# djukic14/BlockSparseMatrices.jl

Hardware: AMD Instinct MI355X
Metric: fp64 block-SpMV GB/s (VBCRS mul!, algorithmic bytes / time) (higher is better)
Workload: dtype f64

## Files before the change

blocksparsematrices.jl_amd/csrc/bsm_analysis.cpp:

```cpp
#include "bsm_analysis.h"

#include <algorithm>
#include <cassert>
#include <chrono>
#include <cmath>
#include <cstdio>
#include <cstdlib>
#include <cstring>
#include <numeric>
#include <set>
#include <thread>
#include <tuple>
#include <unordered_map>

namespace bsm {

Tunables Tunables::from_env() {
    Tunables t;
    auto geti = [](const char *name, int64_t dflt) -> int64_t {
        const char *s = std::getenv(name);
        if (!s || !*s) return dflt;
        return std::strtoll(s, nullptr, 10);
    };
    t.split2_bytes = geti("BSM_SPLIT2_BYTES", t.split2_bytes);
// ... 207 lines not shown
struct Item {
    int64_t group;
    int64_t s_begin, s_end;
    int64_t bytes;
    int nw;
    int32_t color;
};

struct C64h {
    float re, im;
};
struct C128h {
    double re, im;
};
template <typename U> inline const U &stored(const U &v) { return v; }
inline float stored(double v) { return (float)v; }
inline C64h stored(const C128h &v) { return C64h{(float)v.re, (float)v.im}; }

template <typename U, typename V = U>
void pack_chunk_perm(const V *src, int64_t ld, int ra, int mc, int64_t n, const int32_t *dstpos, int E,
                     bool trans, U *dst) {
    for (int64_t w = 0; w < n; w++) {
        const int64_t mp = dstpos[w];
        U *d = dst + ((mp / E) * mc) * E + (mp % E);
        if (!trans) {
            const V *col = src + ra + w * ld;
            for (int i = 0; i < mc; i++) d[(int64_t)i * E] = stored(col[i]);
        } else {
            const V *row = src + w + (int64_t)ra * ld;
            for (int i = 0; i < mc; i++) d[(int64_t)i * E] = stored(row[(int64_t)i * ld]);
        }
    }
}

template <typename U, typename V = U>
void pack_chunk(const V *src, int64_t ld, int ra, int mc, int64_t n, int64_t woff, int E, bool trans,
                U *dst) {
    const int64_t s_first = woff / E, s_last = (woff + n - 1) / E;
    for (int64_t s = s_first; s <= s_last; s++) {
        const int64_t w0 = s * E - woff;
        const int e_lo = (int)std::max<int64_t>(0, -w0);
        const int e_hi = (int)std::min<int64_t>(E, n - w0);
        U *d = dst + (s * mc) * E;
        if (!trans) {
            for (int e = e_lo; e < e_hi; e++) {
                const V *col = src + ra + (w0 + e) * ld;
                for (int i = 0; i < mc; i++) d[(int64_t)i * E + e] = stored(col[i]);
            }
        } else {
            for (int i = 0; i < mc; i++) {
                const V *row = src + w0 + (int64_t)(ra + i) * ld;
                for (int e = e_lo; e < e_hi; e++) d[(int64_t)i * E + e] = stored(row[e]);
            }
        }
    }
}

struct U16 {
    uint64_t a, b;
};

uint64_t hash_list(const int64_t *p, int64_t n) {
    uint64_t h = 0xcbf29ce484222325ull ^ (uint64_t)n;
    for (int64_t i = 0; i < n; i++) {
        h ^= (uint64_t)p[i];
        h *= 0x100000001b3ull;
        h ^= h >> 29;
    }
    return h;
}

}

namespace {
int64_t count_scale_waves(const std::vector<uint8_t> &cover, int64_t own_lo, int64_t own_hi);
}

struct Analysis::BuildState {
    bool sym = false;
    bool colored = false;
    int64_t nb = 0;
    int64_t own_lo = 0, own_hi = 0;
    std::vector<Chunk> chunks;
    std::vector<Group> groups;
    std::vector<const int64_t *> glist;
    std::vector<int32_t> colpos;
    std::vector<uint8_t> ckind;
    std::vector<uint8_t> group_perm;
    std::vector<int64_t> layout;
    uint64_t val_units = 0;
    std::vector<uint8_t> cover;
    std::vector<int32_t> group_color;
    int32_t ncolors_fused = 1;
    std::vector<Item> items;
    bool use_window = false;
    std::unordered_map<uint64_t, int32_t> cuts;
    std::vector<int64_t> item_wg;
    int64_t nwg_items = 0;
    std::vector<int64_t> wg_perm;
};

std::string Analysis::build(int mtype_, int dtype_, int64_t nrows_, int64_t ncols_,
                            const std::vector<BlockIn> &blocks, const AnalysisOptions &opt_) {
    mtype = mtype_;
    dtype = dtype_;
    nrows = nrows_;
    ncols = ncols_;
    opt = opt_;
    tun = Tunables::from_env();
    const bool timing = std::getenv("BSM_TIMING") != nullptr;
    auto t_last = std::chrono::steady_clock::now();
    auto lap = [&](const char *what) {
        if (!timing) return;
        auto now = std::chrono::steady_clock::now();
        std::fprintf(stderr, "[bsm analysis] %-28s %8.1f ms\n", what,
                     std::chrono::duration<double, std::milli>(now - t_last).count());
        t_last = now;
    };
    BuildState st;
    std::string err = stage_validate(blocks, st);
    if (!err.empty()) return err;
    lap("validate");
    bool colour_oom = false;
    if (opt.meta_only) {
        reference_colourings(blocks, colour_oom);
        return colour_oom ? "out of host memory (colouring)" : "";
    }
    if (!(err = stage_row_groups(blocks, st)).empty()) return err;
    if (!(err = stage_merge_columns(blocks, st)).empty()) return err;
    lap("groups + column lists");
    if (!(err = stage_accumulation(blocks, st)).empty()) return err;
    lap("exclusivity / fused colours");
    std::thread colour_thread([&] { reference_colourings(blocks, colour_oom); });
    struct Joiner {
        std::thread &t;
        ~Joiner() {
            if (t.joinable()) t.join();
        }
    } colour_join{colour_thread};
    stage_work_items(st);
    if (plan_cuts(st)) {
        if (!(err = stage_row_groups(blocks, st)).empty()) return err;
        if (!(err = stage_merge_columns(blocks, st)).empty()) return err;
        if (!(err = stage_accumulation(blocks, st)).empty()) return err;
        stage_work_items(st);
        assert(st.nwg_items + (count_scale_waves(st.cover, st.own_lo, st.own_hi) + kWavesPerWg - 1) / kWavesPerWg <= resident_capacity());
        lap("row cuts: groups again");
    }
    stage_dispatch_order(st);
    stage_place_values(st);
    lap("work items + value placement");
    if (!(err = stage_pack_values(blocks, st)).empty()) return err;
    lap("pack values");
    stage_waves(st);
    stage_windows(st);
    if (!(err = stage_gather_index(st)).empty()) return err;
    lap("schedule");
    colour_thread.join();
    lap("reference colourings (tail not hidden by packing)");
    if (colour_oom) return "out of host memory (colouring)";
    return "";
}

std::string Analysis::stage_validate(const std::vector<BlockIn> &blocks, BuildState &st) {
    static const int kEs[6] = {4, 8, 8, 16, 4, 8};
    static const int kVs[6] = {4, 8, 8, 16, 8, 16};
    if (dtype < 0 || dtype > 5) return "unknown dtype";
    es = kEs[dtype];
    vs = kVs[dtype];
    E = 16 / es;
    if (nrows < 0 || ncols < 0) return "negative matrix size";
    if (nrows > INT32_MAX - 64 || ncols > INT32_MAX - 64) return "matrix dimension exceeds int32 range";
    const int64_t nb = st.nb = (int64_t)blocks.size();
    bool sym = (mtype == MT_SYMMETRIC);
    for (const BlockIn &B : blocks) sym |= (B.kind != KIND_PLAIN);
    st.sym = sym;
    st.own_lo = (opt.own_lo > 0) ? opt.own_lo - 1 : 0;
    st.own_hi = (opt.own_hi > 0) ? std::min(opt.own_hi, nrows) : nrows;
    const int64_t rlim = sym ? std::min(nrows, ncols) : nrows;
    const int64_t clim = sym ? std::min(nrows, ncols) : ncols;

    nnz = 0;
    stored_entries = 0;
    int64_t idx_meta = 0;
    for (int64_t b = 0; b < nb; b++) {
        const BlockIn &B = blocks[b];
        if (B.m < 0 || B.n < 0) return "block " + std::to_string(b + 1) + ": negative size";
        if (B.m > 0 && B.n > 0 && !B.data) return "block " + std::to_string(b + 1) + ": null data";
        if (B.ld < std::max<int64_t>(B.trans ? B.n : B.m, 1))
            return "block " + std::to_string(b + 1) + ": ld < m";
        if (B.m > 0 && !B.ridx && (B.r0 < 1 || B.r0 + B.m - 1 > rlim))
            return "block " + std::to_string(b + 1) + ": row range outside matrix";
        if (B.n > 0 && !B.cidx && (B.c0 < 1 || B.c0 + B.n - 1 > clim))
            return "block " + std::to_string(b + 1) + ": column range outside matrix";
        if (opt.validate) {
            if (B.ridx)
                for (int64_t i = 0; i < B.m; i++)
                    if (B.ridx[i] < 1 || B.ridx[i] > rlim)
                        return "block " + std::to_string(b + 1) + ": row index out of range";
            if (B.cidx)
                for (int64_t i = 0; i < B.n; i++)
                    if (B.cidx[i] < 1 || B.cidx[i] > clim)
                        return "block " + std::to_string(b + 1) + ": column index out of range";
        }
        stored_entries += B.m * B.n;
        nnz += (B.kind == KIND_OFF ? 2 : 1) * B.m * B.n;
        idx_meta += (B.kind == KIND_DIAG) ? B.m : (B.m + B.n);
    }
    {
        int64_t meta;
        if (mtype == MT_VBCRS)
            meta = 8 * ((int64_t)rowptr.size() + (int64_t)rowindices.size() + 4 * nb);
        else
            meta = 8 * idx_meta;
        alg_bytes = stored_entries * es + meta + ncols * vs + nrows * vs;
    }

    return "";
}

void Analysis::reference_colourings(const std::vector<BlockIn> &blocks, bool &colour_oom) {
    const int64_t nb = (int64_t)blocks.size();
    {
        try {
            for (auto &c : colors) c.clear();
            if (opt.skip_colors) return;
            auto refcolor = [&](const std::vector<const int64_t *> &l, const std::vector<int64_t> &n) {
                return opt.coloring == 1 ? color_dsatur(l, n) : color_workstream_dsatur(l, n);
            };
            auto single = [](int64_t n) {
                std::vector<std::vector<int64_t>> out(1);
                out[0].resize(n);
                std::iota(out[0].begin(), out[0].end(), (int64_t)1);
                return out;
            };
            if (mtype == MT_BLOCKSPARSE) {
                if (opt.scheduler == 0) {
                    colors[0] = single(nb);
                    colors[1] = single(nb);
                } else {
                    std::vector<const int64_t *> rl(nb), cl(nb);
                    std::vector<int64_t> rn(nb), cn(nb);
                    for (int64_t b = 0; b < nb; b++) {
                        rl[b] = blocks[b].ridx;
                        rn[b] = blocks[b].ridx ? blocks[b].m : 0;
                        cl[b] = blocks[b].cidx;
                        cn[b] = blocks[b].cidx ? blocks[b].n : 0;
                    }
                    colors[0] = refcolor(rl, rn);
                    colors[1] = refcolor(cl, cn);
                }
            } else if (mtype == MT_SYMMETRIC) {
                std::vector<const int64_t *> dl, rl, cl;
                std::vector<int64_t> dn, rn, cn;
                for (const BlockIn &B : blocks) {
                    if (B.kind == KIND_DIAG) {
                        dl.push_back(B.ridx);
                        dn.push_back(B.ridx ? B.m : 0);
                    } else {
                        rl.push_back(B.ridx);
                        rn.push_back(B.ridx ? B.m : 0);
                        cl.push_back(B.cidx);
                        cn.push_back(B.cidx ? B.n : 0);
                    }
                }
                colors[0] = refcolor(rl, rn);
                colors[1] = refcolor(cl, cn);
                colors[2] = refcolor(dl, dn);
            }
        } catch (const std::bad_alloc &) {
            colour_oom = true;
        }
    }
}

std::string Analysis::stage_row_groups(const std::vector<BlockIn> &blocks, BuildState &st) {
    const int64_t nb = st.nb;
    auto &chunks = st.chunks;
    auto &groups = st.groups;
    auto &glist = st.glist;
    const int chunk_rows = tun.chunk_rows;
    std::unordered_map<uint64_t, std::vector<int64_t>> gmap;

    chunks.clear();
    groups.clear();
    glist.clear();
    rows.clear();
    cols.clear();
    for (int64_t b = 0; b < nb; b++) {
        const BlockIn &B = blocks[b];
        if (B.m == 0 || B.n == 0) continue;
        for (int64_t ra0 = 0; ra0 < B.m; ra0 += chunk_rows) {
            const int mc0 = (int)std::min<int64_t>(chunk_rows, B.m - ra0);
            int cut_h = mc0;
            if (!st.cuts.empty() && B.kind == KIND_PLAIN) {
                bool contig = true;
                if (B.ridx)
                    for (int i = 1; i < mc0 && contig; i++) contig = B.ridx[ra0 + i] == B.ridx[ra0] + i;
                if (contig) {
                    const int64_t rb = (B.ridx ? B.ridx[ra0] : B.r0 + ra0) - 1;
                    auto it = st.cuts.find(((uint64_t)rb << 8) | (uint64_t)mc0);
                    if (it != st.cuts.end()) cut_h = it->second;
                }
            }
            for (int64_t ra = ra0; ra < ra0 + mc0; ra += cut_h) {
                const int mc = (int)std::min<int64_t>(cut_h, ra0 + mc0 - ra);
                bool rcontig = true;
// ... 385 lines not shown
        }
        if (best == load[a]) break;
        const int64_t d = cost[mine[a][bi]] - cost[mine[bc][bj]];
        std::swap(mine[a][bi], mine[bc][bj]);
        load[a] -= d;
        load[bc] += d;
    }
    st.wg_perm.assign((size_t)nwg, -1);
    for (size_t c = 0; c < (size_t)ncus; c++) {
        std::stable_sort(mine[c].begin(), mine[c].end(), [&](int64_t a, int64_t b) { return cost[a] > cost[b]; });
        for (size_t i = 0; i < mine[c].size(); i++) st.wg_perm[(size_t)slots[c][i]] = mine[c][i];
    }
}

void Analysis::stage_place_values(BuildState &st) {
    auto &groups = st.groups;
    std::vector<uint8_t> placed(groups.size(), 0);
    st.layout.clear();
    st.layout.reserve(groups.size());
    std::vector<const Item *> order;
    order.reserve(st.items.size());
    if (st.wg_perm.empty()) {
        for (const Item &it : st.items) order.push_back(&it);
    } else {
        std::vector<std::vector<const Item *>> of_wg(st.wg_perm.size());
        for (size_t i = 0; i < st.items.size(); i++) of_wg[(size_t)st.item_wg[i]].push_back(&st.items[i]);
        for (int64_t w : st.wg_perm) order.insert(order.end(), of_wg[(size_t)w].begin(), of_wg[(size_t)w].end());
    }
    for (const Item *it : order)
        if (!placed[it->group]) {
            placed[it->group] = 1;
            st.layout.push_back(it->group);
        }
    for (size_t g = 0; g < groups.size(); g++)
        if (!placed[g]) st.layout.push_back((int64_t)g);
    uint64_t off = 0;
    for (int64_t g : st.layout) {
        groups[g].val_off = off;
        off += (uint64_t)groups[g].mc * (uint64_t)groups[g].strips;
    }
}

std::string Analysis::stage_pack_values(const std::vector<BlockIn> &blocks, BuildState &st) {
    auto &chunks = st.chunks;
    auto &groups = st.groups;
    auto &colpos = st.colpos;
    auto &group_perm = st.group_perm;
    const uint64_t val_units = st.val_units;

    auto pack_one = [&](const Chunk &c, char *dst) {
        const BlockIn &B = blocks[c.blk];
        if (group_perm[c.group]) {
            const int32_t *dp = colpos.data() + groups[c.group].col_off + c.woff;
            if (dtype == 4)
                pack_chunk_perm<float, double>((const double *)B.data, B.ld, c.ra, c.mc, B.n, dp, E, B.trans, (float *)dst);
            else if (dtype == 5)
                pack_chunk_perm<C64h, C128h>((const C128h *)B.data, B.ld, c.ra, c.mc, B.n, dp, E, B.trans, (C64h *)dst);
            else if (es == 4)
                pack_chunk_perm<uint32_t>((const uint32_t *)B.data, B.ld, c.ra, c.mc, B.n, dp, E, B.trans, (uint32_t *)dst);
            else if (es == 8)
                pack_chunk_perm<uint64_t>((const uint64_t *)B.data, B.ld, c.ra, c.mc, B.n, dp, E, B.trans, (uint64_t *)dst);
            else
                pack_chunk_perm<U16>((const U16 *)B.data, B.ld, c.ra, c.mc, B.n, dp, E, B.trans, (U16 *)dst);
            return;
        }
        if (dtype == 4)
            pack_chunk<float, double>((const double *)B.data, B.ld, c.ra, c.mc, B.n, c.woff, E, B.trans, (float *)dst);
        else if (dtype == 5)
            pack_chunk<C64h, C128h>((const C128h *)B.data, B.ld, c.ra, c.mc, B.n, c.woff, E, B.trans, (C64h *)dst);
        else if (es == 4)
            pack_chunk<uint32_t>((const uint32_t *)B.data, B.ld, c.ra, c.mc, B.n, c.woff, E, B.trans, (uint32_t *)dst);
        else if (es == 8)
            pack_chunk<uint64_t>((const uint64_t *)B.data, B.ld, c.ra, c.mc, B.n, c.woff, E, B.trans, (uint64_t *)dst);
        else
            pack_chunk<U16>((const U16 *)B.data, B.ld, c.ra, c.mc, B.n, c.woff, E, B.trans, (U16 *)dst);
    };
    auto pack_many = [&](const std::vector<int32_t> *ids, size_t nchunks, char *base, size_t wbase) {
        const int nt = (int)std::max<int64_t>(1, std::min<int64_t>(tun.pack_threads, (int64_t)nchunks / 64 + 1));
        auto worker = [&](int t) {
            for (size_t k = t; k < nchunks; k += nt) {
                const Chunk &c = chunks[ids ? (size_t)(*ids)[k] : k];
                pack_one(c, base + ((size_t)groups[c.group].val_off * 16 - wbase));
            }
        };
        std::vector<std::thread> th;
        for (int t = 1; t < nt; t++) th.emplace_back(worker, t);
        worker(0);
        for (auto &x : th) x.join();
    };
    auto zero_tail = [&](const Group &G, char *base, size_t wbase) {
        if (G.strips * E - G.width > 0)
            std::memset(base + (((size_t)G.val_off + (size_t)(G.strips - 1) * G.mc) * 16 - wbase), 0, (size_t)G.mc * 16);
    };
    bool streamed = false;
    pack_plan.clear();
    pack_colpos.clear();
    if (opt.blocks_on_device) {
        pack_plan.reserve(chunks.size());
        bool any_perm = false;
        for (const Chunk &c : chunks) {
            const BlockIn &B = blocks[c.blk];
            PackChunk pc;
            pc.src = (uint64_t)(uintptr_t)B.data;
            pc.dst_unit = groups[c.group].val_off;
            pc.ld = B.ld;
            pc.ra = c.ra;
            pc.mc = c.mc;
            pc.n = (int32_t)B.n;
            pc.woff = (int32_t)c.woff;
            pc.perm_off = group_perm[c.group] ? (int32_t)(groups[c.group].col_off + c.woff) : -1;
            pc.trans = B.trans ? 1 : 0;
            any_perm |= pc.perm_off >= 0;
            pack_plan.push_back(pc);
        }
        if (any_perm) pack_colpos = colpos;
    } else if (opt.sink) {
        std::string err = opt.sink->begin((size_t)value_bytes, &streamed);
        if (!err.empty()) return err;
    }
    if (opt.blocks_on_device) {
    } else if (streamed) {
        const std::vector<int64_t> &lay = st.layout;
        std::vector<int32_t> ids;
        size_t g0 = 0;
        while (g0 < lay.size()) {
            const size_t wbase = (size_t)groups[lay[g0]].val_off * 16;
            size_t g1 = g0, wbytes = 0;
            while (g1 < lay.size() && (g1 == g0 || wbytes + (size_t)groups[lay[g1]].mc * groups[lay[g1]].strips * 16 <= tun.window_bytes)) {
                wbytes += (size_t)groups[lay[g1]].mc * (size_t)groups[lay[g1]].strips * 16;
                g1++;
            }
            char *buf = opt.sink->window(wbytes);
            if (!buf) return "value sink: no staging buffer";
            ids.clear();
            for (size_t g = g0; g < g1; g++) {
                zero_tail(groups[lay[g]], buf, wbase);
                ids.insert(ids.end(), groups[lay[g]].chunks.begin(), groups[lay[g]].chunks.end());
            }
            pack_many(&ids, ids.size(), buf, wbase);
            std::string err = opt.sink->commit(wbase, wbytes);
            if (!err.empty()) return err;
            g0 = g1;
        }
        std::string err = opt.sink->end();
        if (!err.empty()) return err;
    } else {
        values.allocate((size_t)val_units * 16);
        for (const Group &G : groups) zero_tail(G, values.data(), 0);
        pack_many(nullptr, chunks.size(), values.data(), 0);
    }
    return "";
}

void Analysis::stage_waves(BuildState &st) {
    auto &groups = st.groups;
    auto &ckind = st.ckind;
    auto &cover = st.cover;
    auto &items = st.items;
    const bool colored = st.colored;
    const int32_t ncolors_fused = st.ncolors_fused;
    const int64_t own_lo = st.own_lo, own_hi = st.own_hi;

    waves.clear();
    std::vector<WaveWork> *nop_out = &waves;
    auto emit_nop = [&]() {
        WaveWork w;
        std::memset(&w, 0, sizeof w);
        w.work = WORK_NOP;
        w.grp = 1;
        w.rbase = -1;
        nop_out->push_back(w);
    };
    color_wg_ptr.clear();
    int32_t cur_color = -1;
    std::vector<WaveWork> *out = &waves;
    auto item_waves = [&](const Item &it) {
        std::vector<WaveWork> &waves = *out;
        while ((int)(waves.size() % kWavesPerWg) % it.nw != 0) emit_nop();
        const Group &G = groups[it.group];
        const int64_t total = it.s_end - it.s_begin;
        const int64_t per_wave = (total + it.nw - 1) / it.nw;
        for (int w = 0; w < it.nw; w++) {
            const int64_t wa = it.s_begin + std::min<int64_t>(total, (int64_t)w * per_wave);
            const int64_t wb = it.s_begin + std::min<int64_t>(total, (int64_t)(w + 1) * per_wave);
            WaveWork W;
            std::memset(&W, 0, sizeof W);
            W.work = WORK_PANEL;
            W.m = (uint16_t)G.mc;
            W.grp = (uint8_t)it.nw;
            W.lead = (w == 0) ? 1 : 0;
            W.rbase = G.rbase;
            W.row_off = G.row_off;
            W.npieces = 0;
            W.first.kind = G.kind | (G.has_off ? kKindGroupHasOff : 0);
            if (wb > wa) {
                Piece &P = W.first;
                const int64_t c0 = wa * E;
                const int64_t c1 = std::min<int64_t>(G.width, wb * E);
                P.val_off = G.val_off + (uint64_t)wa * (uint64_t)G.mc;
                P.nstrips = (int32_t)(wb - wa);
                P.ncols = (int32_t)(c1 - c0);
                P.col_off = (int32_t)(G.col_off + c0);
                int nseg = 1;
                int32_t segw[3] = {0, P.ncols, P.ncols};
                int32_t segx[3] = {cols[G.col_off + c0], 0, 0};
                int32_t segk[3] = {ckind[G.col_off + c0], 0, 0};
                bool piece_off = ckind[G.col_off + c0] == KIND_OFF;
                for (int64_t k = c0 + 1; k < c1; k++) {
                    piece_off |= ckind[G.col_off + k] == KIND_OFF;
                    if (nseg <= 3 && (cols[G.col_off + k] != cols[G.col_off + k - 1] + 1 ||
                                      ckind[G.col_off + k] != ckind[G.col_off + k - 1])) {
                        if (nseg < 3) {
                            segw[nseg] = (int32_t)(k - c0);
                            segx[nseg] = cols[G.col_off + k];
                            segk[nseg] = ckind[G.col_off + k];
                        }
                        nseg++;
                    }
                }
                if (nseg <= 3) {
                    P.xbase = segx[0];
                    W.seg1_w = segw[1];
                    W.seg1_x = segx[1];
                    W.seg2_w = segw[2];
                    P.seg2_x = segx[2];
                    P.kind = segk[0] | (segk[1] << 2) | (segk[2] << 4);
                } else {
                    P.xbase = -1;
                    W.seg1_w = W.seg2_w = P.ncols;
                    P.kind = G.kind;
                }
                if (piece_off) P.kind |= kKindHasOff;
                if (G.has_off) P.kind |= kKindGroupHasOff;
                W.npieces = 1;
            }
            waves.push_back(W);
        }
    };
    for (const Item &it : items) {
        if (colored && it.color != cur_color) {
            while (waves.size() % kWavesPerWg) emit_nop();
            while ((int32_t)color_wg_ptr.size() <= it.color)
                color_wg_ptr.push_back((int64_t)waves.size() / kWavesPerWg);
            cur_color = it.color;
        }
        item_waves(it);
        assert(colored || (int64_t)(waves.size() - (size_t)it.nw) / kWavesPerWg == st.item_wg[(size_t)(&it - items.data())]);
    }
    while (waves.size() % kWavesPerWg) emit_nop();
    nwg_main = (int64_t)waves.size() / kWavesPerWg;
    assert(colored || nwg_main == st.nwg_items);
    const bool snake = tun.wg_order != 0 && exclusive_fwd;
    if (!st.wg_perm.empty()) {
        assert((int64_t)st.wg_perm.size() == nwg_main);
        std::vector<WaveWork> re(waves.size());
        for (int64_t k = 0; k < nwg_main; k++)
            for (int w = 0; w < kWavesPerWg; w++) re[k * kWavesPerWg + w] = waves[st.wg_perm[k] * kWavesPerWg + w];
        waves.swap(re);
    } else if (!colored && snake && nwg_main > 2) {
        std::vector<WaveWork> re(waves.size());
        const int64_t blk = 256;
        int64_t k = 0;
        for (int64_t a0 = 0; a0 < nwg_main; a0 += blk) {
            const int64_t a1 = std::min(nwg_main, a0 + blk);
            for (int64_t j = 0; j < a1 - a0; j++, k++) {
                const int64_t src = ((a0 / blk) & 1) ? a1 - 1 - j : a0 + j;
                for (int w = 0; w < kWavesPerWg; w++) re[k * kWavesPerWg + w] = waves[src * kWavesPerWg + w];
            }
        }
        waves.swap(re);
    }
    if (colored) {
        while ((int32_t)color_wg_ptr.size() <= ncolors_fused) color_wg_ptr.push_back(nwg_main);
    }

    if (exclusive_fwd) {
        int64_t r = own_lo;
        while (r < own_hi) {
            if (cover[r]) {
                r++;
                continue;
            }
            int64_t e = r;
            while (e < own_hi && !cover[e] && e - r < kScaleRowsPerWave) e++;
            WaveWork W;
            std::memset(&W, 0, sizeof W);
            W.work = WORK_SCALE;
            W.grp = 1;
            W.rbase = (int32_t)r;
            W.first.ncols = (int32_t)(e - r);
            waves.push_back(W);
            r = e;
        }
        while (waves.size() % kWavesPerWg) emit_nop();
    }
    nwg_total = (int64_t)waves.size() / kWavesPerWg;
    auto mark_sync = [](std::vector<WaveWork> &ws) {
        for (size_t wg = 0; wg + kWavesPerWg <= ws.size(); wg += kWavesPerWg) {
            uint8_t sync = 0;
            for (int w = 0; w < kWavesPerWg; w++) sync |= (ws[wg + w].work == WORK_PANEL && ws[wg + w].grp > 1);
            for (int w = 0; w < kWavesPerWg; w++) ws[wg + w].wg_sync = sync;
        }
    };
    mark_sync(waves);

    waves_multi.clear();
    nwg_multi = 0;
    if (tun.multi_wave_bytes > 0 && !exclusive_fwd && !colored && !gather) {
        const int64_t Wm = tun.multi_wave_bytes;
        std::vector<Item> mi;
        for (int64_t g : st.layout) {
            const Group &G = groups[g];
            if (G.strips <= 0) continue;
            const int64_t strip_bytes = (int64_t)G.mc * 16;
            const int64_t maxs = std::max<int64_t>(1, 4 * Wm / strip_bytes);
            const int64_t nitem = (G.strips + maxs - 1) / maxs;
            const int64_t per_item = (G.strips + nitem - 1) / nitem;
            for (int64_t s = 0; s < G.strips; s += per_item) {
                Item it;
                it.group = g;
                it.s_begin = s;
                it.s_end = std::min(G.strips, s + per_item);
                it.bytes = (it.s_end - it.s_begin) * strip_bytes;
                it.nw = it.bytes >= 3 * Wm ? 4 : (it.bytes >= Wm ? 2 : 1);
                it.color = 0;
                mi.push_back(it);
            }
        }
        std::stable_sort(mi.begin(), mi.end(), [](const Item &a, const Item &b) { return a.nw > b.nw; });
        out = nop_out = &waves_multi;
        for (const Item &it : mi) item_waves(it);
        while (waves_multi.size() % kWavesPerWg) emit_nop();
        out = nop_out = &waves;
        size_t panel_main = 0, panel_multi = 0;
        for (const WaveWork &w : waves) panel_main += w.work == WORK_PANEL;
        for (const WaveWork &w : waves_multi) panel_multi += w.work == WORK_PANEL;
        if (4 * panel_multi > 3 * panel_main) {
            waves_multi.clear();
        } else {
            mark_sync(waves_multi);
            nwg_multi = (int64_t)waves_multi.size() / kWavesPerWg;
        }
    }
    if (rows.empty()) rows.push_back(0);
    if (cols.empty()) cols.push_back(0);
    if (values.empty()) {
        values.allocate(16);
        std::memset(values.data(), 0, 16);
    }
}

void Analysis::stage_windows(BuildState &st) {
    auto &ckind = st.ckind;
    const bool use_window = st.use_window;
    win_emissions = win_inside = win_flushed = 0;

    if (use_window) {
        const int64_t cap = window_entries(vs);
        std::vector<int64_t> em;
        win_emissions = win_inside = win_flushed = 0;
        for (size_t wg = 0; wg + kWavesPerWg <= (size_t)nwg_main * kWavesPerWg; wg += kWavesPerWg) {
            int npanel = 0;
            int32_t first_rbase = INT32_MIN, first_rowoff = INT32_MIN;
            bool distinct = false;
            em.clear();
            for (int w = 0; w < kWavesPerWg; w++) {
                const WaveWork &W = waves[wg + w];
                if (W.work != WORK_PANEL || W.npieces == 0) continue;
                if (npanel == 0) {
                    first_rbase = W.rbase;
                    first_rowoff = W.row_off;
                } else if (W.rbase != first_rbase || W.row_off != first_rowoff) {
                    distinct = true;
                }
                npanel++;
                if (W.lead)
                    for (int i = 0; i < W.m; i++) em.push_back((W.rbase >= 0) ? (int64_t)W.rbase + i : rows[W.row_off + i]);
                for (int32_t k = 0; k < W.first.ncols; k++)
                    if (ckind[(size_t)W.first.col_off + k] == KIND_OFF) em.push_back(cols[W.first.col_off + k]);
            }
            win_emissions += (int64_t)em.size();
            if (!distinct || em.empty()) continue;
            std::sort(em.begin(), em.end());
            size_t best_j = 0, best_k = 0, j = 0;
            for (size_t k = 0; k < em.size(); k++) {
                while (em[k] - em[j] >= cap) j++;
                if (k - j > best_k - best_j || k == 0) best_j = j, best_k = k;
            }
            const int64_t inside = (int64_t)(best_k - best_j + 1);
            int64_t uniq = 1;
            for (size_t k = best_j + 1; k <= best_k; k++) uniq += em[k] != em[k - 1];
            if (inside < 32 || 5 * uniq > 4 * inside) continue;
            const int64_t lo = em[best_j], span = em[best_k] - lo + 1;
            for (int w = 0; w < kWavesPerWg; w++) {
                waves[wg + w].win_base = (int32_t)lo;
                waves[wg + w].win_span8 = (uint8_t)((span + 7) / 8);
            }
            win_inside += inside;
            win_flushed += uniq;
        }
    }
}

std::string Analysis::stage_gather_index(BuildState &st) {
    auto &groups = st.groups;
    auto &ckind = st.ckind;

    inv_ptr[0].clear();
    inv_ptr[1].clear();
    inv_idx[0].clear();
    inv_idx[1].clear();
    ws_fbase = ws_slots = 0;
    if (gather) {
        ws_fbase = (int64_t)cols.size();
        int64_t nf = 0;
        for (WaveWork &W : waves) {
            if (W.work != WORK_PANEL || !W.lead) continue;
            W.win_base = (int32_t)nf;
            nf += W.m;
        }
        ws_slots = ws_fbase + nf;
        if (ws_slots + 8 > INT32_MAX) return "gather workspace exceeds int32 slots";
        const int64_t ylen[2] = {nrows, ncols};
        for (int k = 0; k < 2; k++) {
            std::vector<int64_t> ptr((size_t)ylen[k] + 1, 0);
            auto visit = [&](auto &&emit) {
                for (const Group &G : groups)
                    for (int64_t q = 0; q < G.width; q++)
                        if (k == 1 || ckind[G.col_off + q] == KIND_OFF) emit(cols[G.col_off + q], G.col_off + q);
                for (const WaveWork &W : waves) {
                    if (W.work != WORK_PANEL || !W.lead) continue;
                    const bool fwd = (k == 0) || (W.first.kind & kKindGroupHasOff);
                    if (!fwd) continue;
                    for (int i = 0; i < W.m; i++) {
                        const int64_t r = (W.rbase >= 0) ? (int64_t)W.rbase + i : rows[W.row_off + i];
                        emit(r, ws_fbase + W.win_base + i);
                    }
                }
            };
            visit([&](int64_t yi, int64_t) {
                if (yi < ylen[k]) ptr[yi + 1]++;
            });
            for (int64_t j = 0; j < ylen[k]; j++) ptr[j + 1] += ptr[j];
            std::vector<int32_t> csr((size_t)ptr[ylen[k]] + 1, 0);
            {
                std::vector<int64_t> fill(ptr.begin(), ptr.end() - 1);
                visit([&](int64_t yi, int64_t slot) {
                    if (yi < ylen[k]) csr[fill[yi]++] = (int32_t)slot;
                });
            }
            const int64_t ntiles = (ylen[k] + 63) / 64;
            std::vector<int64_t> &tp = inv_ptr[k];
            tp.assign((size_t)ntiles + 1, 0);
            for (int64_t t = 0; t < ntiles; t++) {
                int64_t kmax = 0;
                for (int64_t j = t * 64; j < std::min(ylen[k], (t + 1) * 64); j++)
                    kmax = std::max(kmax, ptr[j + 1] - ptr[j]);
                tp[t + 1] = tp[t] + kmax;
            }
            if (tp[ntiles] * 64 + 64 > INT32_MAX) return "gather index exceeds int32";
            inv_idx[k].assign((size_t)tp[ntiles] * 64 + 64, -1);
            for (int64_t t = 0; t < ntiles; t++)
                for (int64_t j = t * 64; j < std::min(ylen[k], (t + 1) * 64); j++)
                    for (int64_t c = ptr[j]; c < ptr[j + 1]; c++)
                        inv_idx[k][(size_t)(tp[t] + (c - ptr[j])) * 64 + (size_t)(j - t * 64)] = csr[c];
        }
    }
    for (const Group &G : groups)
        if (G.has_off && G.has_diag)
            for (int64_t q = 0; q < G.width; q++)
                if (ckind[G.col_off + q] == KIND_DIAG) cols[G.col_off + q] = (int32_t)((uint32_t)cols[G.col_off + q] | kColDiagBit);
    return "";
}

std::vector<int64_t> Analysis::vbcrs_bookkeeping(int64_t nblocks, const int64_t *rowstart,
                                                 const int64_t *colstart) {
    std::vector<int64_t> p(nblocks);
    std::iota(p.begin(), p.end(), (int64_t)0);
    std::stable_sort(p.begin(), p.end(), [&](int64_t a, int64_t b) {
        if (rowstart[a] != rowstart[b]) return rowstart[a] < rowstart[b];
        return colstart[a] < colstart[b];
    });
    perm.resize(nblocks);
    colindices.resize(nblocks);
    rowptr.clear();
    rowindices.clear();
    rowptr.push_back(1);
    rowindices.push_back(rowstart[p[0]]);
    for (int64_t out = 0; out < nblocks; out++) {
        const int64_t in = p[out];
        if (rowstart[in] != rowindices.back()) {
            rowptr.push_back(out + 1);
            rowindices.push_back(rowstart[in]);
        }
        perm[out] = in + 1;
        colindices[out] = colstart[in];
    }
    rowptr.push_back(nblocks + 1);
    return p;
}

}
// ... 1 lines not shown
```

blocksparsematrices.jl_amd/csrc/bsm_analysis.h:

```cpp
#pragma once
#include <cstdint>
#include <string>
#include <vector>

#include "bsm_layout.h"

namespace bsm {

class RawBuffer {
  public:
    RawBuffer() = default;
    RawBuffer(const RawBuffer &) = delete;
    RawBuffer &operator=(const RawBuffer &) = delete;
    ~RawBuffer() { release(); }
    void allocate(size_t n) {
        release();
        p_ = n ? static_cast<char *>(::operator new(n)) : nullptr;
        n_ = n;
    }
    void release() {
        if (p_) ::operator delete(p_);
        p_ = nullptr;
        n_ = 0;
    }
    char *data() { return p_; }
    const char *data() const { return p_; }
    size_t size() const { return n_; }
    bool empty() const { return n_ == 0; }
    const char &operator[](size_t i) const { return p_[i]; }

  private:
    char *p_ = nullptr;
    size_t n_ = 0;
};

enum MatType { MT_VBCRS = 0, MT_BLOCKSPARSE = 1, MT_SYMMETRIC = 2 };

struct BlockIn {
    const char *data;
    int64_t m, n, ld;
    const int64_t *ridx;
    const int64_t *cidx;
    int64_t r0, c0;
    int kind;
    bool trans = false;
};

struct Tunables {
    int64_t wave_bytes = 0;
    int64_t target_waves = 32768;
    double fat_fill_below = 0.9;
    int64_t wave_bytes_min = 8 << 10, wave_bytes_max = 24 << 10;
    int64_t multi_wave_bytes = 64 << 10;
    int64_t split2_bytes = 0;
    int64_t split4_bytes = 0;
    int64_t wgitem_max_bytes = 0;
    int chunk_rows = kMaxRowsPerChunk;
    int64_t deep_group_bytes = 128 << 10;
    int64_t deep_total_bytes = 64 << 20;
    int pack_threads = 8;
    size_t window_bytes = 64u << 20;
    int lds_window = 1;
    int wg_order = -1;
    int wg_cap_pct = 150;
    int64_t resident_wgs = 0;
    static Tunables from_env();
};

struct ValueSink {
    virtual ~ValueSink() = default;
    virtual std::string begin(size_t total_bytes, bool *use) = 0;
    virtual char *window(size_t bytes) = 0;
    virtual std::string commit(size_t offset, size_t bytes) = 0;
    virtual std::string end() = 0;
};

struct AnalysisOptions {
    int scheduler = 0;
    int validate = 1;
    int accumulate = 0;
    int64_t own_lo = 0, own_hi = 0;
    ValueSink *sink = nullptr;
    bool blocks_on_device = false;
    int coloring = 0;
    bool meta_only = false;
    bool skip_colors = false;
    int num_cus = 0;
};

std::vector<std::vector<int64_t>> color_dsatur(const std::vector<const int64_t *> &lists,
                                               const std::vector<int64_t> &lens);
std::vector<std::vector<int64_t>> color_workstream_dsatur(const std::vector<const int64_t *> &lists,
                                                          const std::vector<int64_t> &lens);

struct PackChunk {
    uint64_t src;
    uint64_t dst_unit;
    int64_t ld;
    int32_t ra, mc;
    int32_t n, woff;
    int32_t perm_off;
    int32_t trans;
};
static_assert(sizeof(PackChunk) == 48, "PackChunk must be 48 bytes");

class Analysis {
  public:
    int mtype = 0, dtype = 0;
    int es = 8;
    int vs = 8;
    int E = 2;
    int64_t nrows = 0, ncols = 0;
    AnalysisOptions opt;
    Tunables tun;

    std::vector<int64_t> perm, rowptr, colindices, rowindices;
    std::vector<std::vector<int64_t>> colors[3];
    int64_t nnz = 0, stored_entries = 0, alg_bytes = 0;

    RawBuffer values;
    std::vector<PackChunk> pack_plan;
    std::vector<int32_t> pack_colpos;
    int64_t value_bytes = 0;
    std::vector<int32_t> rows, cols;
    std::vector<WaveWork> waves;
    std::vector<WaveWork> waves_multi;
    int64_t nwg_multi = 0;
    double lane_fill = 1.0;
    double mean_rows = 64.0;
    int64_t nwg_main = 0;
    int64_t nwg_total = 0;
    int64_t ngroups = 0;
    bool exclusive_fwd = false;
    std::vector<int64_t> color_wg_ptr;
    int64_t win_emissions = 0, win_inside = 0, win_flushed = 0;
    bool gather = false;
    int64_t ws_fbase = 0, ws_slots = 0;
    std::vector<int64_t> inv_ptr[2];
    std::vector<int32_t> inv_idx[2];

    std::string build(int mtype, int dtype, int64_t nrows, int64_t ncols,
                      const std::vector<BlockIn> &blocks, const AnalysisOptions &opt);

    std::vector<int64_t> vbcrs_bookkeeping(int64_t nblocks, const int64_t *rowstart, const int64_t *colstart);

  private:
    struct BuildState;
    std::string stage_validate(const std::vector<BlockIn> &blocks, BuildState &st);
    void reference_colourings(const std::vector<BlockIn> &blocks, bool &colour_oom);
    std::string stage_row_groups(const std::vector<BlockIn> &blocks, BuildState &st);
    std::string stage_merge_columns(const std::vector<BlockIn> &blocks, BuildState &st);
    std::string stage_accumulation(const std::vector<BlockIn> &blocks, BuildState &st);
    void stage_work_items(BuildState &st);
    int64_t resident_capacity() const;
    bool plan_cuts(BuildState &st);
    void stage_dispatch_order(BuildState &st);
    void stage_place_values(BuildState &st);
    std::string stage_pack_values(const std::vector<BlockIn> &blocks, BuildState &st);
    void stage_waves(BuildState &st);
    void stage_windows(BuildState &st);
    std::string stage_gather_index(BuildState &st);
};

}
```

blocksparsematrices.jl_amd/csrc/bsm_one.hip:

```cpp
#include "bsm_device.h"
#include "bsm_families.h"

namespace bsm {

#ifndef BSM_C64_FUSED_WAVES
#define BSM_C64_FUSED_WAVES 5
#endif
#ifndef BSM_C128_FUSED_WAVES
#define BSM_C128_FUSED_WAVES 6
#endif

template <typename T, int L, int P, bool FWD, bool TRN, bool NT, typename S = T>
__device__ __forceinline__ T run_panel(const WaveD &wd, const uint4 *__restrict__ values,
                                       const int *__restrict__ rows, const int *__restrict__ cols,
                                       const T *__restrict__ x, T *__restrict__ y, T alpha,
                                       int flags, int lane, T *xs, T *vs, T *win, int win_n,
                                       T *__restrict__ ws) {
    constexpr int E = TT<S>::E;
    constexpr int G = 64 / P;
    constexpr int V = L * E;
    constexpr int NC = G * L * E;
    constexpr int XCH = x_chunk_cols<T, TRN>();
    using XV = typename std::conditional<std::is_same<S, T>::value, Vec16<T>, XVec<T, E>>::type;
    constexpr int BF = XCH / NC;
    static_assert(XCH % NC == 0, "x chunk must hold whole iterations");
    constexpr bool INPLACE = FWD && TRN;
    int *ix = reinterpret_cast<int *>(vs);
    const bool opT = (flags & FLAG_OPT) != 0;
    const bool cjf = (flags & FLAG_CONJ) != 0;
    const int m = wd.m;
    const int i = lane & (P - 1);
    const int g = lane / P;
    const bool row_ok = i < m;

    T acc[E];
#pragma unroll
    for (int e = 0; e < E; ++e) acc[e] = zero_of(T{});
    T xr = zero_of(T{});
    if (TRN && row_ok) {
        const int ri = row_index(wd, rows, i);
        xr = x[ri];
    }

    const PieceD pc = wd.first;
    if (wd.npieces > 0) {
        const int xbase = pc.xbase;
        const int col_off = pc.col_off;
        const int nstrips = pc.nstrips;
        const int ncols = pc.ncols;
        const int kinds = pc.kind;
        const bool has_off = (kinds & kKindHasOff) != 0;
        const bool fwd_en = FWD && (!opT || has_off);
        const bool trn_en = TRN && (opT || has_off);
        const Vec16<S> *__restrict__ vb = reinterpret_cast<const Vec16<S> *>(
            values + (((uint64_t)pc.val_hi << 32) | pc.val_lo));
        const int s1w = wd.seg1_w, s1x = wd.seg1_x - wd.seg1_w;
        const int s2w = wd.seg2_w, s2x = pc.seg2_x - wd.seg2_w;
        auto col_lookup = [&](int w, bool &off) -> int {
            if (xbase < 0) {
                const int raw = cols[col_off + w];
                off = raw >= 0 && (kinds & 3) == KIND_OFF;
                return raw & 0x7fffffff;
            }
            const int sh = w < s1w ? 0 : (w < s2w ? 2 : 4);
            off = ((kinds >> sh) & 3) == KIND_OFF;
            return w + (w < s1w ? xbase : (w < s2w ? s1x : s2x));
        };

        auto load_b = [&](Vec16<S>(&b)[L], int s0) {
#pragma unroll
            for (int l = 0; l < L; ++l) {
                const int s = s0 + l * G + g;
                if (row_ok && s < nstrips) {
                    b[l] = NT ? load_stream16(&vb[(uint32_t)(s * m + i)]) : vb[(uint32_t)(s * m + i)];
                } else {
#pragma unroll
                    for (int e = 0; e < E; ++e) b[l].v[e] = zero_of(S{});
                }
            }
        };
        auto stage_x = [&](int c0, auto kx_tag) {
            constexpr int KX = decltype(kx_tag)::value;
            const bool pool = xbase < 0;
            int raw[KX];
            T xv[KX];
            if (pool) {
#pragma unroll
                for (int k = 0; k < KX; ++k) raw[k] = cols[col_off + min(c0 + k * 64 + lane, ncols - 1)];
#pragma unroll
                for (int k = 0; k < KX; ++k) xv[k] = x[raw[k] & 0x7fffffff];
            } else {
#pragma unroll
                for (int k = 0; k < KX; ++k) {
                    bool off;
                    raw[k] = 0;
                    xv[k] = x[col_lookup(min(c0 + k * 64 + lane, ncols - 1), off)];
                }
            }
#pragma unroll
            for (int k = 0; k < KX; ++k) {
                const int w = c0 + k * 64 + lane;
                bool off;
                int yi = raw[k] & 0x7fffffff;
                if (pool)
                    off = raw[k] >= 0 && (kinds & 3) == KIND_OFF;
                else
                    yi = col_lookup(min(w, ncols - 1), off);
                xs[k * 64 + lane] = (w < ncols && (!opT || off)) ? xv[k] : zero_of(T{});
                if (INPLACE) ix[k * 64 + lane] = (w < ncols && (opT || off)) ? yi : -1;
            }
        };

        auto stage_chunk = [&](int c0) {
            if (!fwd_en && !(INPLACE && trn_en)) return;
            if (BSM_DBG(DBG_NO_XGATHER)) {
#pragma unroll
                for (int k = 0; k < XCH / 64; ++k) {
                    xs[k * 64 + lane] = alpha;
                    if (INPLACE) {
                        const int w = c0 + k * 64 + lane;
                        bool off = false;
                        const int yi = col_lookup(min(w, ncols - 1), off);
                        ix[k * 64 + lane] = (w < ncols && (opT || off)) ? yi : -1;
                    }
                }
                return;
            }
            constexpr int KXM = XCH / 64;
            const int need = min(ncols - c0, XCH) + NC;
            if (KXM >= 4 && need <= (KXM / 4) * 64)
                stage_x(c0, std::integral_constant<int, (KXM >= 4 ? KXM / 4 : 1)>{});
            else if (KXM >= 2 && need <= (KXM / 2) * 64)
                stage_x(c0, std::integral_constant<int, (KXM >= 2 ? KXM / 2 : 1)>{});
            else
                stage_x(c0, std::integral_constant<int, KXM>{});
        };
        auto iteration = [&](Vec16<S>(&b)[L], int s0, int c0, int s_end) {
            if (fwd_en) {
                const int cb = (s0 - c0 / E) * E;
#pragma unroll
                for (int l = 0; l < L; ++l) {
                    const XV xv = *reinterpret_cast<const XV *>(&xs[cb + (l * G + g) * E]);
#pragma unroll
                    for (int e = 0; e < E; ++e) acc[e] = madd(acc[e], widen(T{}, cj(b[l].v[e], cjf)), xv.v[e]);
                }
            }
#ifdef BSM_TRACE
            if (s0 == 0) {
                asm volatile("s_waitcnt vmcnt(0)" ::: "memory");
                BSM_TSTAMP(3);
            }
#endif
            if (trn_en) {
                T vals[V];
#pragma unroll
                for (int l = 0; l < L; ++l)
#pragma unroll
                    for (int e = 0; e < E; ++e) vals[l * E + e] = mul(widen(T{}, cj(b[l].v[e], cjf)), xr);
                int pos = 0, dup = 0;
                if (!BSM_DBG(DBG_NO_BUTTERFLY)) Butterfly<T, V, P>::run(vals, i, pos, dup);
                constexpr int CF = (V / P) > 1 ? (V / P) : 1;
                const int slot = (s0 - c0 / E) / (G * L);
                T *park = INPLACE ? xs : vs;
                if ((i & dup) == 0) {
#pragma unroll
                    for (int j = 0; j < CF; ++j) {
                        const int q = pos + j;
                        const int l = q / E, e = q % E;
                        park[slot * NC + (l * G + g) * E + e] = vals[j];
                    }
                }
                const bool last_it = (s0 + G * L >= s_end);
                if ((slot == BF - 1 || last_it) && !BSM_DBG(DBG_NO_EMISSION)) {
                    const int sb = s0 - slot * (G * L);
                    const int nbatch = min((slot + 1) * NC, ncols - sb * E);
#pragma unroll 1
                    for (int k = 0; k * 64 < nbatch; ++k) {
                        const int c = k * 64 + lane;
                        const int w = sb * E + c;
                        if (c < nbatch) {
                            int yi;
                            if (INPLACE) {
                                yi = ix[c];
                                if (yi < 0) continue;
                            } else {
                                bool off;
                                yi = col_lookup(w, off);
                                if (!(opT || off)) continue;
                            }
                            if (flags & FLAG_GATHER) {
                                ws[col_off + w] = park[c];
                                continue;
                            }
                            const T val = mul(alpha, park[c]);
                            const unsigned wi = (unsigned)(yi - wd.win_base);
                            if (wi < (unsigned)win_n) {
                                if (!BSM_DBG(DBG_NO_WINDOW_ADD)) lds_acc(&win[wi], val);
                            } else if (flags & FLAG_RMW) {
                                y[yi] = add(y[yi], val);
                            } else if (!BSM_DBG(DBG_NO_GLOBAL_ATOMICS)) {
                                atomic_acc(&y[yi], val);
                            }
                        }
                    }
                }
            }
        };

        for (int c0 = 0; c0 < ncols; c0 += XCH) {
            stage_chunk(c0);
#ifdef BSM_TRACE
            if (c0 == 0) BSM_TSTAMP(2);
#endif
            const int s_end = min(nstrips, (c0 + XCH) / E);
            for (int s0 = c0 / E; s0 < s_end; s0 += G * L) {
                Vec16<S> b[L];
                __builtin_amdgcn_s_setprio(3);
                load_b(b, s0);
                __builtin_amdgcn_s_setprio(0);
                iteration(b, s0, c0, s_end);
            }
        }
    }
    T a = acc[0];
    if (FWD) {
#pragma unroll
        for (int e = 1; e < E; ++e) a = add(a, acc[e]);
#pragma unroll
        for (int d = P; d < 64; d <<= 1) a = add(a, shx(a, d));
    }
    return a;
}

template <typename T, bool FWD, bool TRN> constexpr int kMixedWaves = (FWD && TRN && std::is_same<T, double>::value) ? 7 : 6;
#ifndef BSM_CVEC_WAVES
#define BSM_CVEC_WAVES 6
#endif

template <typename T, int L, bool FWD, bool TRN, bool NT, typename S = T>
__global__ void __launch_bounds__(64 * kWavesPerWg) __attribute__((amdgpu_waves_per_eu(
    kCvec<T, S> ? BSM_CVEC_WAVES :
    !std::is_same<S, T>::value ? kMixedWaves<T, FWD, TRN> :
    (FWD && TRN && (std::is_same<T, double>::value || std::is_same<T, float>::value)) ? 8 :
    (FWD && TRN && std::is_same<T, c128>::value) ? (L == 4 ? 8 : BSM_C128_FUSED_WAVES) :
    (FWD && TRN && std::is_same<T, c64>::value) ? (L == 4 ? 8 : BSM_C64_FUSED_WAVES) :
    (((!TRN && std::is_same<T, double>::value) || std::is_same<T, c128>::value) ? 6 : 5))))
    __attribute__((amdgpu_num_sgpr(96)))
    panel_kernel(const WaveWork *__restrict__ waves, const uint4 *__restrict__ values, const int *__restrict__ rows,
                 const int *__restrict__ cols, const T *__restrict__ x, T *__restrict__ y, T alpha,
                 T beta, int flags, unsigned wg_base, T *__restrict__ ws, long long ws_fbase) {
    constexpr int XS = x_chunk_cols<T, TRN>();
    constexpr int VS = XS;
    __shared__ __attribute__((aligned(16))) T xs[kWavesPerWg][FWD ? XS : 1];
    __shared__ __attribute__((aligned(16))) T vs[kWavesPerWg][TRN ? VS : 1];
    constexpr bool WIN = FWD && TRN;
    __shared__ T win[WIN ? window_entries((int)sizeof(T)) : 1];

    const int wave = __builtin_amdgcn_readfirstlane(threadIdx.x >> 6);
    const int lane = threadIdx.x & 63;
    BSM_TSTAMP(0);
    const WaveD wd = load_wave(waves + ((size_t)(blockIdx.x + wg_base) * kWavesPerWg + wave));
    const int work = wd.work;
    const int m = wd.m;
#ifdef BSM_TRACE
    asm volatile("s_waitcnt lgkmcnt(0)" ::: "memory");
    BSM_TSTAMP(1);
    if (lane == 0) {
        t_trace[threadIdx.x >> 6][6] =
            (unsigned long long)(wd.work == WORK_PANEL && wd.npieces ? (long long)wd.first.nstrips * wd.m * 16 : 0);
        t_trace[threadIdx.x >> 6][7] = wall_clock64();
        t_trace[threadIdx.x >> 6][9] = (unsigned long long)__builtin_amdgcn_s_getreg(BSM_GETREG_HW_ID);
        t_trace[threadIdx.x >> 6][10] = (unsigned long long)__builtin_amdgcn_s_getreg(BSM_GETREG_XCC_ID);
    }
#endif
    int win_n = (WIN && !(flags & FLAG_RMW)) ? wd.win_n : 0;
    if constexpr (kCvec<T, S>) win_n = min(win_n, window_entries((int)sizeof(T)));
    if (WIN && win_n > 0) {
        for (int e = threadIdx.x; e < win_n; e += 64 * kWavesPerWg) win[e] = zero_of(T{});
        __syncthreads();
    }

    T u = zero_of(T{});
    if (work == WORK_PANEL) {
        if (m <= 8)
            u = run_panel<T, L, 8, FWD, TRN, NT, S>(wd, values, rows, cols, x, y, alpha, flags, lane, xs[wave], vs[wave], win, win_n, ws);
        else if (m <= 16)
            u = run_panel<T, L, 16, FWD, TRN, NT, S>(wd, values, rows, cols, x, y, alpha, flags, lane, xs[wave], vs[wave], win, win_n, ws);
        else if (m <= 32)
            u = run_panel<T, L, 32, FWD, TRN, NT, S>(wd, values, rows, cols, x, y, alpha, flags, lane, xs[wave], vs[wave], win, win_n, ws);
        else
            u = run_panel<T, L, 64, FWD, TRN, NT, S>(wd, values, rows, cols, x, y, alpha, flags, lane, xs[wave], vs[wave], win, win_n, ws);
    }
    BSM_TSTAMP(4);
    const bool direct = (flags & FLAG_DIRECT) != 0;
    const bool sz = (flags & FLAG_STRONG_ZERO) != 0;
    if (FWD) {
        if (wd.wg_sync) {
            xs[wave][lane] = u;
            __syncthreads();
        }
        if (work == WORK_PANEL && wd.lead && !BSM_DBG(DBG_NO_FWD_OUT)) {
            for (int k = 1; k < wd.grp; ++k) u = add(u, xs[wave + k][lane]);
            if (flags & FLAG_GATHER) {
                const bool fwd_on = !(flags & FLAG_OPT) || (wd.first.kind & kKindGroupHasOff);
                if (lane < m && fwd_on) ws[ws_fbase + wd.win_base + lane] = u;
            } else if (lane < m) {
                const int yi = row_index(wd, rows, lane);
                const T val = mul(alpha, u);
                const unsigned wi = (unsigned)(yi - wd.win_base);
                if (direct) {
                    y[yi] = sz ? val : madd(val, beta, y[yi]);
                } else if (wi < (unsigned)win_n) {
                    lds_acc(&win[wi], val);
                } else if (flags & FLAG_RMW) {
                    y[yi] = add(y[yi], val);
                } else {
                    atomic_acc(&y[yi], val);
                }
            }
        }
    }
    if (WIN && win_n > 0) {
        __syncthreads();
        for (int e = threadIdx.x; e < win_n; e += 64 * kWavesPerWg) {
            const T v = win[e];
            if (!is_zero(v)) atomic_acc(&y[wd.win_base + e], v);
        }
    }
    if (work == WORK_SCALE && direct) {
        const int cnt = wd.first.ncols;
        for (int r = lane; r < cnt; r += 64)
            y[wd.rbase + r] = sz ? zero_of(T{}) : mul(beta, y[wd.rbase + r]);
    }
#ifdef BSM_TRACE
    asm volatile("s_waitcnt vmcnt(0)" ::: "memory");
    BSM_TSTAMP(5);
    if (lane == 0) t_trace[threadIdx.x >> 6][8] = wall_clock64();
    if (g_trace && lane < 16)
        g_trace[((size_t)blockIdx.x * kWavesPerWg + (threadIdx.x >> 6)) * 16 + lane] = t_trace[threadIdx.x >> 6][lane];
#endif
}

template <typename T>
__global__ void __launch_bounds__(256) scale_kernel(T *__restrict__ y, long long ldy, long long lo,
                                                    long long hi, T beta, int strong_zero) {
    constexpr int E = TT<T>::E;
    T *__restrict__ yc = y + (long long)blockIdx.y * ldy + lo;
    const long long n = hi - lo;
    const long long tid = (long long)blockIdx.x * blockDim.x + threadIdx.x;
    const long long stride = (long long)gridDim.x * blockDim.x;
    const unsigned gap = (unsigned)((16 - ((uintptr_t)yc & 15)) & 15);
    if (gap % sizeof(T)) {
        for (long long i = tid; i < n; i += stride) yc[i] = strong_zero ? zero_of(T{}) : mul(beta, yc[i]);
        return;
    }
    long long head = (long long)(gap / sizeof(T));
    if (head > n) head = n;
    const long long nvec = (n - head) / E;
    Vec16<T> *__restrict__ yv = reinterpret_cast<Vec16<T> *>(yc + head);
    for (long long u = tid; u < nvec; u += stride) {
        Vec16<T> v;
        if (strong_zero) {
#pragma unroll
            for (int e = 0; e < E; ++e) v.v[e] = zero_of(T{});
        } else {
            v = yv[u];
#pragma unroll
            for (int e = 0; e < E; ++e) v.v[e] = mul(beta, v.v[e]);
        }
        yv[u] = v;
    }
    const long long tail0 = head + nvec * E;
    if (tid < head) yc[tid] = strong_zero ? zero_of(T{}) : mul(beta, yc[tid]);
// ... 117 lines not shown
```

Baseline: 6170.

## Use buffer loads for block values and issue first strip loads during x staging

Matrix value loads for non-float, non-transposed paths now go through raw buffer loads with a buffer resource descriptor. Out-of-range strips are handled by hardware bounds checking instead of per-lane branches. For forward f64-style paths, the first strip's value loads are issued inside the x-gather staging, fenced by scheduling barriers, so their latency overlaps with the x gather and LDS writes. A host-side check rejects wave pieces over 2 GiB, since the buffer offset is 32-bit.

```diff
diff --git a/blocksparsematrices.jl_amd/csrc/bsm_analysis.cpp b/blocksparsematrices.jl_amd/csrc/bsm_analysis.cpp
--- a/blocksparsematrices.jl_amd/csrc/bsm_analysis.cpp
+++ b/blocksparsematrices.jl_amd/csrc/bsm_analysis.cpp
@@ -383,7 +383,7 @@
     lap("work items + value placement");
     if (!(err = stage_pack_values(blocks, st)).empty()) return err;
     lap("pack values");
-    stage_waves(st);
+    if (!(err = stage_waves(st)).empty()) return err;
     stage_windows(st);
     if (!(err = stage_gather_index(st)).empty()) return err;
     lap("schedule");
@@ -1075,7 +1075,7 @@
     return "";
 }
 
-void Analysis::stage_waves(BuildState &st) {
+std::string Analysis::stage_waves(BuildState &st) {
     auto &groups = st.groups;
     auto &ckind = st.ckind;
     auto &cover = st.cover;
@@ -1097,6 +1097,7 @@
     color_wg_ptr.clear();
     int32_t cur_color = -1;
     std::vector<WaveWork> *out = &waves;
+    std::string piece_err;
     auto item_waves = [&](const Item &it) {
         std::vector<WaveWork> &waves = *out;
         while ((int)(waves.size() % kWavesPerWg) % it.nw != 0) emit_nop();
@@ -1122,6 +1123,7 @@
                 const int64_t c1 = std::min<int64_t>(G.width, wb * E);
                 P.val_off = G.val_off + (uint64_t)wa * (uint64_t)G.mc;
                 P.nstrips = (int32_t)(wb - wa);
+                if ((wb - wa) * (int64_t)G.mc * 16 >= ((int64_t)1 << 31)) piece_err = "wave piece exceeds 2 GiB";
                 P.ncols = (int32_t)(c1 - c0);
                 P.col_off = (int32_t)(G.col_off + c0);
                 int nseg = 1;
@@ -1170,6 +1172,7 @@
         item_waves(it);
         assert(colored || (int64_t)(waves.size() - (size_t)it.nw) / kWavesPerWg == st.item_wg[(size_t)(&it - items.data())]);
     }
+    if (!piece_err.empty()) return piece_err;
     while (waves.size() % kWavesPerWg) emit_nop();
     nwg_main = (int64_t)waves.size() / kWavesPerWg;
     assert(colored || nwg_main == st.nwg_items);
@@ -1271,6 +1274,7 @@
         values.allocate(16);
         std::memset(values.data(), 0, 16);
     }
+    return "";
 }
 
 void Analysis::stage_windows(BuildState &st) {
diff --git a/blocksparsematrices.jl_amd/csrc/bsm_analysis.h b/blocksparsematrices.jl_amd/csrc/bsm_analysis.h
--- a/blocksparsematrices.jl_amd/csrc/bsm_analysis.h
+++ b/blocksparsematrices.jl_amd/csrc/bsm_analysis.h
@@ -157,7 +157,7 @@
     void stage_dispatch_order(BuildState &st);
     void stage_place_values(BuildState &st);
     std::string stage_pack_values(const std::vector<BlockIn> &blocks, BuildState &st);
-    void stage_waves(BuildState &st);
+    std::string stage_waves(BuildState &st);
     void stage_windows(BuildState &st);
     std::string stage_gather_index(BuildState &st);
 };
diff --git a/blocksparsematrices.jl_amd/csrc/bsm_one.hip b/blocksparsematrices.jl_amd/csrc/bsm_one.hip
--- a/blocksparsematrices.jl_amd/csrc/bsm_one.hip
+++ b/blocksparsematrices.jl_amd/csrc/bsm_one.hip
@@ -8,6 +8,9 @@
 #endif
 #ifndef BSM_C128_FUSED_WAVES
 #define BSM_C128_FUSED_WAVES 6
+#endif
+#ifndef BSM_EARLY_STRIPS
+#define BSM_EARLY_STRIPS 1
 #endif
 
 template <typename T, int L, int P, bool FWD, bool TRN, bool NT, typename S = T>
@@ -25,6 +28,10 @@
     constexpr int BF = XCH / NC;
     static_assert(XCH % NC == 0, "x chunk must hold whole iterations");
     constexpr bool INPLACE = FWD && TRN;
+    constexpr bool BUF = !TRN && !std::is_same<T, float>::value &&
+                         !(std::is_same<T, double>::value && std::is_same<S, float>::value);
+    constexpr bool EARLY = BUF && FWD && BSM_EARLY_STRIPS &&
+                           !(std::is_same<T, c128>::value && (std::is_same<S, c128>::value || std::is_same<S, double>::value));
     int *ix = reinterpret_cast<int *>(vs);
     const bool opT = (flags & FLAG_OPT) != 0;
     const bool cjf = (flags & FLAG_CONJ) != 0;
@@ -67,19 +74,30 @@
             return w + (w < s1w ? xbase : (w < s2w ? s1x : s2x));
         };
 
+        const __amdgpu_buffer_rsrc_t rs =
+            __builtin_amdgcn_make_buffer_rsrc((void *)vb, (short)0, nstrips * m * 16, 0x00020000);
         auto load_b = [&](Vec16<S>(&b)[L], int s0) {
-#pragma unroll
-            for (int l = 0; l < L; ++l) {
-                const int s = s0 + l * G + g;
-                if (row_ok && s < nstrips) {
-                    b[l] = NT ? load_stream16(&vb[(uint32_t)(s * m + i)]) : vb[(uint32_t)(s * m + i)];
-                } else {
-#pragma unroll
-                    for (int e = 0; e < E; ++e) b[l].v[e] = zero_of(S{});
+            if constexpr (BUF) {
+                const unsigned v0 = row_ok ? (unsigned)((s0 + g) * m + i) * 16u : 0x80000000u;
+#pragma unroll
+                for (int l = 0; l < L; ++l) {
+                    const u32x4 r = __builtin_amdgcn_raw_buffer_load_b128(rs, (int)(v0 + (unsigned)(l * G * m * 16)), 0, NT ? 2 : 0);
+                    __builtin_memcpy(&b[l], &r, 16);
+                }
+            } else {
+#pragma unroll
+                for (int l = 0; l < L; ++l) {
+                    const int s = s0 + l * G + g;
+                    if (row_ok && s < nstrips) {
+                        b[l] = NT ? load_stream16(&vb[(uint32_t)(s * m + i)]) : vb[(uint32_t)(s * m + i)];
+                    } else {
+#pragma unroll
+                        for (int e = 0; e < E; ++e) b[l].v[e] = zero_of(S{});
+                    }
                 }
             }
         };
-        auto stage_x = [&](int c0, auto kx_tag) {
+        auto stage_x = [&](int c0, auto kx_tag, auto &&early) {
             constexpr int KX = decltype(kx_tag)::value;
             const bool pool = xbase < 0;
             int raw[KX];
@@ -97,6 +115,9 @@
                     xv[k] = x[col_lookup(min(c0 + k * 64 + lane, ncols - 1), off)];
                 }
             }
+            if constexpr (EARLY) __builtin_amdgcn_sched_barrier(0);
+            early();
+            if constexpr (EARLY) __builtin_amdgcn_sched_barrier(0);
 #pragma unroll
             for (int k = 0; k < KX; ++k) {
                 const int w = c0 + k * 64 + lane;
@@ -111,9 +132,10 @@
             }
         };
 
-        auto stage_chunk = [&](int c0) {
-            if (!fwd_en && !(INPLACE && trn_en)) return;
+        auto stage_chunk = [&](int c0, auto &&early) {
+            if (!fwd_en && !(INPLACE && trn_en)) return early();
             if (BSM_DBG(DBG_NO_XGATHER)) {
+                early();
 #pragma unroll
                 for (int k = 0; k < XCH / 64; ++k) {
                     xs[k * 64 + lane] = alpha;
@@ -129,11 +151,11 @@
             constexpr int KXM = XCH / 64;
             const int need = min(ncols - c0, XCH) + NC;
             if (KXM >= 4 && need <= (KXM / 4) * 64)
-                stage_x(c0, std::integral_constant<int, (KXM >= 4 ? KXM / 4 : 1)>{});
+                stage_x(c0, std::integral_constant<int, (KXM >= 4 ? KXM / 4 : 1)>{}, early);
             else if (KXM >= 2 && need <= (KXM / 2) * 64)
-                stage_x(c0, std::integral_constant<int, (KXM >= 2 ? KXM / 2 : 1)>{});
+                stage_x(c0, std::integral_constant<int, (KXM >= 2 ? KXM / 2 : 1)>{}, early);
             else
-                stage_x(c0, std::integral_constant<int, KXM>{});
+                stage_x(c0, std::integral_constant<int, KXM>{}, early);
         };
         auto iteration = [&](Vec16<S>(&b)[L], int s0, int c0, int s_end) {
             if (fwd_en) {
@@ -207,18 +229,37 @@
             }
         };
 
+        auto request = [&](Vec16<S>(&b)[L], int s0) {
+            __builtin_amdgcn_s_setprio(3);
+            if constexpr (BUF) __builtin_amdgcn_sched_barrier(0);
+            load_b(b, s0);
+            if constexpr (BUF) __builtin_amdgcn_sched_barrier(0);
+            __builtin_amdgcn_s_setprio(0);
+        };
         for (int c0 = 0; c0 < ncols; c0 += XCH) {
-            stage_chunk(c0);
+            const int s_end = min(nstrips, (c0 + XCH) / E);
+            if constexpr (EARLY) {
+                Vec16<S> b[L];
+                int s0 = c0 / E;
+                stage_chunk(c0, [&] { request(b, s0); });
 #ifdef BSM_TRACE
-            if (c0 == 0) BSM_TSTAMP(2);
-#endif
-            const int s_end = min(nstrips, (c0 + XCH) / E);
-            for (int s0 = c0 / E; s0 < s_end; s0 += G * L) {
-                Vec16<S> b[L];
-                __builtin_amdgcn_s_setprio(3);
-                load_b(b, s0);
-                __builtin_amdgcn_s_setprio(0);
+                if (c0 == 0) BSM_TSTAMP(2);
+#endif
                 iteration(b, s0, c0, s_end);
+                for (s0 += G * L; s0 < s_end; s0 += G * L) {
+                    request(b, s0);
+                    iteration(b, s0, c0, s_end);
+                }
+            } else {
+                stage_chunk(c0, [] {});
+#ifdef BSM_TRACE
+                if (c0 == 0) BSM_TSTAMP(2);
+#endif
+                for (int s0 = c0 / E; s0 < s_end; s0 += G * L) {
+                    Vec16<S> b[L];
+                    request(b, s0);
+                    iteration(b, s0, c0, s_end);
+                }
             }
         }
     }
```

New measurement: 6162, median of 4. Within noise of the previous version (-0.1%).
